# CloudEngineHub/PARC

Measured on AMD Instinct MI355X. Metric: env-steps/s, higher is better.
Workload: dtype f32; 1 GPU; full step (dynamics + obs/reward/done), 65536 envs total = 65536 per GPU, 5 bundled clips on a square blocky grid, reset of finished envs included; envs_per_gpu=65536, total_envs=65536, dynamics=True, parallelism=env-shard x1, launch=stream launches, library_abi=6

## Files before the change

parc_amd/csrc/parc_env.hip:

```cpp
#include <hip/hip_runtime.h>

#include <cmath>
#include <cstddef>
#include <cstdio>
#include <cstring>
#include <new>
#include <string>
#include <vector>

#include "../../include/parc_env.h"
#include "parc_common.hpp"
#include "parc_math.hpp"
#include "parc_dynamics.hpp"
#include "parc_dynamics_coop.hpp"
#include "parc_dynamics_wave.hpp"

using namespace parc;

#define REC_F4 32
#define REC_Q_POS 15
#define REC_Q_CONTACT 16
#define REC_Q_VEL 20

struct HierTables {
    float lt[16][3];
    float lr[16][4];
    int fk_paths[PARC_MAX_FK_PATHS][PARC_MAX_FK_DEPTH];
    int key_ids[8];
    int key_slot[16];
    int parent[16];
    int jtype[16];
    int dof_idx[16];
    float axis[16][4];
};
#define HIER_STAGED_WORDS ((int)(offsetof(HierTables, parent) / 4))

#define TILE_MAX_CELLS 320

struct DevTables {
    HierTables h;
    float tstep[8];
    float joint_err_w[16];
    float dof_err_w[PARC_MAX_DOFS];
    float contact_w[16];
    float pose_term_dist[16];
};

struct StepParams {
    int N, B, J, D, K, S, R, M, T;
    int lds_wave_floats;
    int global_obs, off_char;
    int lr_identity;
    int obs_tar, obs_contact;
    int obs_dim, off_dofvel, off_key, off_tar, tar_w, off_tarc, off_cc, off_hf;
    float dt_f, episode_length, min_obs_h, max_obs_h;
    float pose_w, vel_w, root_pos_w, root_vel_w, key_pos_w;
    float root_pos_term_sq, root_rot_term;
    int early_term, pose_term, track_root, track_root_h, tracking, body_pos_from_fk, never_done;
    unsigned fall_mask;
    float term_h;
    const float *hf; int X, Y; float min_x, min_y, dx, dy; int tile_r;
    float rdx, rdy;
    unsigned tile_mul;
    float tstep[8];
    const float4 *records; const MotionMeta *meta; const float *motion_offsets; const float *env_offsets;
    const float *ray_points; const DevTables *tables;
    unsigned char *ema_code;
    unsigned *stamp_out;
    float4 *prep;
    ParcEnvBuffers buf;
};

__device__ __forceinline__ Q4 joint_dof_to_rot(int type, const float *axis4, const float *dof) {
    if (type == PARC_JOINT_HINGE) return axis_angle_to_quat(mk3(axis4[0], axis4[1], axis4[2]), dof[0]);
    if (type == PARC_JOINT_SPHERICAL) return exp_map_to_quat(mk3(dof[0], dof[1], dof[2]));
    return mk4(0.f, 0.f, 0.f, 1.f);
}

__device__ __forceinline__ void joint_rot_to_dof(int type, const float *axis4, Q4 q, float *out) {
    if (type == PARC_JOINT_HINGE) {
        V3 axis; float angle;
        quat_to_axis_angle(q, axis, angle);
        float dot = axis4[0] * axis.x + axis4[1] * axis.y + axis4[2] * axis.z;
        if (dot < 0.f) angle = angle * -1.f;
        out[0] = angle;
    } else if (type == PARC_JOINT_SPHERICAL) {
        V3 e = quat_to_exp_map(q);
        out[0] = e.x; out[1] = e.y; out[2] = e.z;
    }
}

__device__ __forceinline__ float cell_float_rcp(float p, float mn, float d, float rd) {
    const float x = p - mn;
    const float q0 = x * rd;
    const float r = fmaf(-d, q0, x);
    return rintf(fmaf(r, rd, q0));
}
__device__ __forceinline__ int cell_index_rcp(float p, float mn, float d, float rd) {
    float f = cell_float_rcp(p, mn, d, rd);
    f = fminf(fmaxf(f, -1.0e9f), 1.0e9f);
    return (int)f;
}

__device__ __forceinline__ int cell_index(float p, float mn, float d) {
    float f = rintf((p - mn) / d);
    f = fminf(fmaxf(f, -1.0e9f), 1.0e9f);
    return (int)f;
}

__global__ __launch_bounds__(64) void k_dynamics(const parcdyn::DynModel *__restrict__ M, parcdyn::DynTerrain T, ParcEnvBuffers buf,
                                                 const float *__restrict__ action, const float *__restrict__ env_off, int N) {
    const int e = blockIdx.x * blockDim.x + threadIdx.x;
    if (e >= N) return;
    parcdyn::DynState S;
    S.root_pos = buf.char_root_pos + 3 * (size_t)e; S.root_rot = buf.char_root_rot + 4 * (size_t)e;
    S.root_vel = buf.char_root_vel + 3 * (size_t)e; S.root_ang_vel = buf.char_root_ang_vel + 3 * (size_t)e;
    S.dof_pos = buf.char_dof_pos + (size_t)M->D * e; S.dof_vel = buf.char_dof_vel + (size_t)M->D * e;
    S.contact_force = buf.contact_forces + (size_t)3 * M->B * e; S.body_pos = nullptr;
    parcdyn::dyn_control_step(*M, T, S, action + (size_t)M->D * e, env_off + 3 * (size_t)e);
}

__global__ __launch_bounds__(64) void k_env_prep(const StepParams P, const int64_t *__restrict__ env_ids,
                                                 const int *__restrict__ env_ids32, const int *__restrict__ count_dev, int count) {
    if (count_dev) count = *count_dev;
    const int it = blockIdx.x * 4 + (threadIdx.x >> 4), j = threadIdx.x & 15;
    if (it >= count || j >= P.B) return;
    const int e = env_ids ? (int)env_ids[it] : (env_ids32 ? env_ids32[it] : it);
    const DevTables *__restrict__ T = P.tables;
    float4 *out = P.prep + (size_t)e * 16;
    if (j == 0) {
        const float4 rr = *(const float4 *)(P.buf.char_root_rot + 4 * (size_t)e);
        const float heading = calc_heading(rr);
        const Q4 hinv = heading_quat_inv(heading);
        out[0] = make_float4(cosf(heading), sinf(heading), hinv.z, hinv.w);
    } else {
        const float *dof = P.buf.char_dof_pos + (size_t)e * P.D;
        const int ty = T->h.jtype[j], di = T->h.dof_idx[j];
        Q4 q = mk4(0.f, 0.f, 0.f, 1.f);
        if (ty == PARC_JOINT_HINGE) q = axis_angle_to_quat(mk3(T->h.axis[j][0], T->h.axis[j][1], T->h.axis[j][2]), dof[di]);
        else if (ty == PARC_JOINT_SPHERICAL) q = exp_map_to_quat(mk3(dof[di], dof[di + 1], dof[di + 2]));
        out[j] = q;
    }
}

#ifdef PARC_STAMPS
#define STAMP(i) do { if (lane == 0) s_stamp[i] = __builtin_readcyclecounter(); } while (0)
#else
#define STAMP(i) do { } while (0)
#endif
#define MODE_STEP 0
#define MODE_OBS 1
#define ENVS_PER_BLOCK 4
#define WAVE_SYNC() asm volatile("" ::: "memory")
#define RAY_UNROLL 8

__device__ __forceinline__ float wave_sum(float v) {
#pragma unroll
    for (int off = 32; off >= 1; off >>= 1) v = v + __shfl_xor(v, off, 64);
    return v;
}

template <int CTRL>
__device__ __forceinline__ float dpp_f32(float v) {
    return __int_as_float(__builtin_amdgcn_update_dpp(0, __float_as_int(v), CTRL, 0xf, 0xf, false));
}
__device__ __forceinline__ float row_sum16(float v) {
    v = v + dpp_f32<0x128>(v);
    v = v + dpp_f32<0x124>(v);
    v = v + dpp_f32<0x122>(v);
    v = v + dpp_f32<0x121>(v);
    return v;
}
__device__ __forceinline__ float lane_value(float v, int l) { return __int_as_float(__builtin_amdgcn_readlane(__float_as_int(v), l)); }

template <int MODE, bool MIRROR, bool LOCALROOT = false, bool OBSVAR = false>
__global__ __launch_bounds__(256, 5) void k_env_post(const StepParams P, const int64_t *__restrict__ env_ids,
                                                 const int *__restrict__ env_ids32, const int *__restrict__ count_dev, int count,
                                                 unsigned long long *bump_calls) {
    extern __shared__ __align__(16) float s_obs_all[];
    __shared__ int s_tab_raw[HIER_STAGED_WORDS];
    const HierTables &s_tab = *reinterpret_cast<const HierTables *>(s_tab_raw);
    __shared__ float4 s_q_all[ENVS_PER_BLOCK][8][16];
    __shared__ float4 s_lq_all[ENVS_PER_BLOCK][2][16];
    __shared__ float4 s_fk_all[ENVS_PER_BLOCK][80];
    __shared__ float s_cdofv_all[ENVS_PER_BLOCK][PARC_MAX_DOFS];
    __shared__ float4 s_refvel_all[ENVS_PER_BLOCK][12];
    __shared__ float s_refct_all[ENVS_PER_BLOCK][16];
    __shared__ float s_cfn_all[ENVS_PER_BLOCK][16];
    __shared__ float s_sc_all[ENVS_PER_BLOCK][16];
#ifdef PARC_STAMPS
    __shared__ unsigned long long s_stamp_all[ENVS_PER_BLOCK][16];
#endif
    const int wv = __builtin_amdgcn_readfirstlane((int)(threadIdx.x >> 6));
    const int lane = threadIdx.x & 63;
    const bool GLOBALOBS = OBSVAR && P.global_obs != 0;
    const int oc = OBSVAR ? P.off_char : 0;
    const bool TAROBS = !OBSVAR || P.obs_tar != 0;
    const bool CONTACTOBS = !OBSVAR || P.obs_contact != 0;
    float *s_obs = s_obs_all + (size_t)wv * P.lds_wave_floats;
    float4 (*s_q)[16] = s_q_all[wv];
    float4 (*s_lq)[16] = s_lq_all[wv];
    float4 *s_fk = s_fk_all[wv];
    float4 *s_cbp = s_lq[0];
    float *s_cdofv = s_cdofv_all[wv];
    float4 *s_refvel = s_refvel_all[wv];
    float *s_refct = s_refct_all[wv], *s_cfn = s_cfn_all[wv];
#ifdef PARC_STAMPS
    unsigned long long *s_stamp = s_stamp_all[wv];
#endif
    float *s_tile = (float *)s_fk;
    float4 (*s_br)[16] = reinterpret_cast<float4 (*)[16]>(s_obs + ((P.off_tarc + 3) & ~3));

    if (MODE == MODE_OBS && bump_calls && blockIdx.x == 0 && threadIdx.x == 0) *bump_calls += 1ull;
    if (count_dev) count = *count_dev;
    const int it = blockIdx.x * ENVS_PER_BLOCK + wv;
    if (it >= count) return;
    int e = env_ids ? (int)env_ids[it] : (env_ids32 ? env_ids32[it] : it);
    e = __builtin_amdgcn_readfirstlane(e);
    STAMP(0);

    const int B = P.B, D = P.D, S = P.S, K = P.K, J = P.J;
    const DevTables *__restrict__ T = P.tables;

    float *orow = P.buf.obs + (size_t)e * P.obs_dim;

    constexpr int HW = HIER_STAGED_WORDS;
    constexpr int HN = (HW + 63) / 64;
    int tabreg[HN];
#pragma unroll
    for (int i = 0; i < HN; ++i) { const int w = lane + 64 * i; tabreg[i] = w < HW ? ((const int *)&T->h)[w] : 0; }
    float dofv = 0.f;
    if (lane < D) dofv = P.buf.char_dof_vel[(size_t)e * D + lane];
    float aux0 = 0.f, aux1 = 0.f, aux2 = 0.f;
    {
        const float *src = nullptr;
        if (lane >= 32 && lane < 32 + B) src = P.buf.contact_forces + 3 * ((size_t)e * B + (lane - 32));
        else if (lane == 30) src = P.buf.char_root_vel + 3 * (size_t)e;
        else if (lane == 31) src = P.buf.char_root_ang_vel + 3 * (size_t)e;
        if (src) { aux0 = src[0]; aux1 = src[1]; aux2 = src[2]; }
    }
    const int qi = lane & 15;
    float4 prepq = make_float4(0.f, 0.f, 0.f, 1.f);
    if (lane < 16) prepq = P.prep[(size_t)e * 16 + lane];
    float2 rayp[RAY_UNROLL];
#pragma unroll
    for (int i = 0; i < RAY_UNROLL; ++i) {
        const int r = lane + 64 * i;
        rayp[i] = r < P.R ? ((const float2 *)P.ray_points)[r] : make_float2(0.f, 0.f);
    }

    const int mid = P.buf.motion_ids[e];
    const int tid = P.buf.terrain_ids[e];
    const float toff = P.buf.time_offsets[e];
    int ts = P.buf.timestep[e];
    if (MODE == MODE_STEP) ts += 1;
    const float time = P.dt_f * (float)ts;
    const float mt = time + toff;
    const MotionMeta meta = P.meta[mid];
    const float eox = P.env_offsets[3 * e + 0], eoy = P.env_offsets[3 * e + 1], eoz = P.env_offsets[3 * e + 2];
    const float *mo = P.motion_offsets + 2 * ((size_t)mid * P.T + tid);
    const float offx = mo[0] - eox, offy = mo[1] - eoy;
    const float *crp = P.buf.char_root_pos + 3 * (size_t)e;
    const float *crr = P.buf.char_root_rot + 4 * (size_t)e;
    const V3 root_pos = mk3(crp[0], crp[1], crp[2]);
    const Q4 root_rot = mk4(crr[0], crr[1], crr[2], crr[3]);
    const float gx = root_pos.x + eox, gy = root_pos.y + eoy, gz = root_pos.z + eoz;

    Blend myb;
    {
        const int sid = lane & 7;
        float t = mt;
#pragma unroll
        for (int q = 0; q < PARC_MAX_TAR_STEPS; ++q) t = (sid - 1 == q) ? mt + P.tstep[q] : t;
        myb = frame_blend(meta, t);
    }
    const int last_frame = meta.start + meta.nframes - 1;
    float4 fA[2], fB[2];
    Blend bl[2];
#pragma unroll
    for (int p = 0; p < 2; ++p) {
        const int r = p * 4 + (lane >> 4);
        const int src = max(r - 1, 0);
        bl[p].b = __shfl(myb.b, src, 64);
        bl[p].i0 = __shfl(myb.i0, src, 64);
        bl[p].i1 = min(bl[p].i0 + 1, last_frame);
        fA[p] = make_float4(0.f, 0.f, 0.f, 1.f); fB[p] = fA[p];
        if (r >= 1 && r < 2 + S) {
            fA[p] = P.records[(size_t)bl[p].i0 * REC_F4 + qi];
            fB[p] = P.records[(size_t)bl[p].i1 * REC_F4 + qi];
        }
    }
    float4 cA = make_float4(0.f, 0.f, 0.f, 0.f), cB = cA;
    float cblend = 0.f;
    const int nvel = 2 + (D + 3) / 4;
    {
        const int src = lane < 4 * (1 + S) ? lane >> 2 : 0;
        const float b2b = __shfl(myb.b, src, 64);
        const int b2i0 = __shfl(myb.i0, src, 64), b2i1 = min(b2i0 + 1, last_frame);
        if (lane < 4 * (1 + S)) {
            const int c = lane & 3;
            cblend = b2b;
            cA = P.records[(size_t)b2i0 * REC_F4 + REC_Q_CONTACT + c];
            cB = P.records[(size_t)b2i1 * REC_F4 + REC_Q_CONTACT + c];
        } else if (lane >= 32 && lane < 32 + nvel) {
            cA = P.records[(size_t)b2i0 * REC_F4 + REC_Q_VEL + (lane - 32)];
        }
    }
    const int tr = P.tile_r, TW = 2 * tr + 1, ncell = tr >= 0 ? TW * TW : 0;
    const int ox = min(max(cell_index(gx, P.min_x, P.dx) - tr, -(1 << 22)), 1 << 22), oy = min(max(cell_index(gy, P.min_y, P.dy) - tr, -(1 << 22)), 1 << 22);
    float tilev[5];
#pragma unroll
    for (int i = 0; i < 5; ++i) {
        const int idx = lane + 64 * i;
        tilev[i] = 0.f;
        if (idx < ncell) {
            const int a = (int)(((unsigned)idx * P.tile_mul) >> 16), bq = idx - a * TW;
            const int cx = min(max(ox + a, 0), P.X - 1), cy = min(max(oy + bq, 0), P.Y - 1);
            tilev[i] = P.hf[(size_t)cx * P.Y + cy];
        }
    }

    const float ch = __shfl(prepq.x, 0, 64), sh = __shfl(prepq.y, 0, 64);
    const Q4 hinv = mk4(0.f, 0.f, __shfl(prepq.z, 0, 64), __shfl(prepq.w, 0, 64));
#pragma unroll
    for (int i = 0; i < HN; ++i) { const int w = lane + 64 * i; if (w < HW) s_tab_raw[w] = tabreg[i]; }
    if (lane < D) {
        s_cdofv[lane] = dofv;
        s_obs[P.off_dofvel + lane] = dofv;
    }
    if (OBSVAR && oc && lane == 29) s_obs[0] = root_pos.z;
    if (lane == 30 || lane == 31) {
        const V3 r = GLOBALOBS ? mk3(aux0, aux1, aux2) : quat_rotate(hinv, mk3(aux0, aux1, aux2));
        const int o = oc + (lane == 30 ? 6 : 9);
        s_obs[o + 0] = r.x; s_obs[o + 1] = r.y; s_obs[o + 2] = r.z;
    }
    if (lane >= 32 && lane < 32 + B) {
        const float n = norm3(mk3(aux0, aux1, aux2));
        if (CONTACTOBS) orow[P.off_cc + (lane - 32)] = n > 1e-5f ? 1.f : 0.f;
        s_cfn[lane - 32] = fminf(n, 1.0f);
    }
#pragma unroll
    for (int i = 0; i < 5; ++i) { const int idx = lane + 64 * i; if (idx < ncell) s_tile[idx] = tilev[i]; }
    WAVE_SYNC();
    STAMP(1);

    {
        float *hrow = orow + P.off_hf;
        float *hmirror = MIRROR && P.buf.ray_hfs ? P.buf.ray_hfs + (size_t)e * P.R : nullptr;
        for (int base = 0; base < P.R; base += 64 * RAY_UNROLL) {
            if (base > 0) {
#pragma unroll
                for (int i = 0; i < RAY_UNROLL; ++i) { const int r = base + lane + 64 * i; rayp[i] = r < P.R ? ((const float2 *)P.ray_points)[r] : make_float2(0.f, 0.f); }
            }
            const float tlox = (float)ox, thix = (float)(ox + TW - 1), tloy = (float)oy, thiy = (float)(oy + TW - 1);
            if (tr >= 0) {
                int tix[RAY_UNROLL];
#pragma unroll
                for (int i = 0; i < RAY_UNROLL; ++i) {
                    tix[i] = 0;
                    if (base + 64 * i < P.R) {
                        const float px = (rayp[i].x * ch - rayp[i].y * sh) + gx;
                        const float py = (rayp[i].x * sh + rayp[i].y * ch) + gy;
                        const int a = (int)fminf(fmaxf(cell_float_rcp(px, P.min_x, P.dx, P.rdx), tlox), thix) - ox;
                        const int bq = (int)fminf(fmaxf(cell_float_rcp(py, P.min_y, P.dy, P.rdy), tloy), thiy) - oy;
                        tix[i] = a * TW + bq;
                    }
                    asm volatile("" : "+v"(tix[i]));
                }
                float hv[RAY_UNROLL];
#pragma unroll
                for (int i = 0; i < RAY_UNROLL; ++i) hv[i] = s_tile[tix[i]];
#pragma unroll
                for (int i = 0; i < RAY_UNROLL; ++i) {
                    const int r = base + lane + 64 * i;
                    if (r < P.R) {
                        float h = hv[i] - gz;
                        h = fminf(fmaxf(h, P.min_obs_h), P.max_obs_h);
                        hrow[r] = h;
                        if (hmirror) hmirror[r] = h;
                    }
                }
            } else {
#pragma unroll
                for (int i = 0; i < RAY_UNROLL; ++i) {
                    const int r = base + lane + 64 * i;
                    if (r < P.R) {
                        const float px = (rayp[i].x * ch - rayp[i].y * sh) + gx;
                        const float py = (rayp[i].x * sh + rayp[i].y * ch) + gy;
                        const int ix = cell_index_rcp(px, P.min_x, P.dx, P.rdx), iy = cell_index_rcp(py, P.min_y, P.dy, P.rdy);
                        const int cx = min(max(ix, 0), P.X - 1), cy = min(max(iy, 0), P.Y - 1);
                        float h = P.hf[(size_t)cx * P.Y + cy] - gz;
                        h = fminf(fmaxf(h, P.min_obs_h), P.max_obs_h);
                        hrow[r] = h;
                        if (hmirror) hmirror[r] = h;
                    }
                }
            }
        }
    }
    STAMP(2);

#pragma unroll
    for (int p = 0; p < 2; ++p) {
        const int r = p * 4 + (lane >> 4);
        const int i = qi;
        if (r < 2 + S) {
            float4 res = make_float4(0.f, 0.f, 0.f, 1.f);
            if (r == 0) {
                if (i == 0) res = root_rot;
                else if (i == 15) res = make_float4(root_pos.x, root_pos.y, root_pos.z, 0.f);
                else if (i < B) res = prepq;
            } else {
                const float4 A = fA[p], Bv = fB[p];
                const float bb = bl[p].b;
                if (i == 15) {
                    const float a = 1.0f - bb;
                    res.x = a * A.x + bb * Bv.x;
                    res.y = a * A.y + bb * Bv.y;
                    res.z = a * A.z + bb * Bv.z;
                    res.w = 0.f;
                    if (meta.loop == PARC_LOOP_WRAP) {
                        float t = mt;
#pragma unroll
                        for (int q = 0; q < PARC_MAX_TAR_STEPS; ++q) t = (r - 2 == q) ? mt + P.tstep[q] : t;
                        const float ph = floorf(t / meta.length);
                        res.x = res.x + ph * meta.dx; res.y = res.y + ph * meta.dy; res.z = res.z + ph * meta.dz;
                    }
                    res.x = res.x + offx;
                    res.y = res.y + offy;
                } else if (i < B) {
                    res = slerp_rr(A, Bv, bb);
                }
            }
            if (i >= 1 && i < B) {
                const Q4 lq = P.lr_identity ? res : quat_mul(mk4(s_tab.lr[i][0], s_tab.lr[i][1], s_tab.lr[i][2], s_tab.lr[i][3]), res);
                if (r < 2) { s_lq[r][i] = lq; s_q[r][i] = res; } else s_q[r][i] = lq;
            } else {
                s_q[r][i] = res;
            }
            if (r == 1) {
                if (MIRROR && i == 0 && P.buf.ref_root_rot) *(float4 *)(P.buf.ref_root_rot + 4 * (size_t)e) = res;
                if (MIRROR && i >= 1 && i < B && P.buf.ref_joint_rot) *(float4 *)(P.buf.ref_joint_rot + 4 * ((size_t)e * J + i - 1)) = res;
                if (MIRROR && i == 15 && P.buf.ref_root_pos) {
                    float *o = P.buf.ref_root_pos + 3 * (size_t)e;
                    o[0] = res.x; o[1] = res.y; o[2] = res.z;
                }
            } else if (r == 0 || TAROBS) {
                const int base = r == 0 ? 0 : P.off_tar + (r - 2) * P.tar_w;
                if (i < B) {
                    const Q4 qq = (i == 0 && !GLOBALOBS) ? quat_mul(hinv, res) : res;
                    float tn[6];
                    quat_to_tan_norm(qq, tn);
                    const int o = r == 0 ? oc + (i == 0 ? 0 : 12 + 6 * (i - 1)) : base + 3 + 6 * i;
#pragma unroll
                    for (int c = 0; c < 6; ++c) s_obs[o + c] = tn[c];
                } else if (i == 15 && r >= 2) {
                    const V3 rpd = mk3(res.x - root_pos.x, res.y - root_pos.y, res.z - root_pos.z);
                    const V3 rpo = GLOBALOBS ? rpd : quat_rotate(hinv, rpd);
                    s_obs[base + 0] = rpo.x; s_obs[base + 1] = rpo.y; s_obs[base + 2] = rpo.z;
                }
            }
        }
    }
    if (lane < 4 * (1 + S)) {
        const int s = lane >> 2, c = lane & 3;
        const float b = cblend, a = 1.0f - b;
        const float v[4] = {a * cA.x + b * cB.x, a * cA.y + b * cB.y, a * cA.z + b * cB.z, a * cA.w + b * cB.w};
#pragma unroll
        for (int k = 0; k < 4; ++k) {
            const int bd = 4 * c + k;
            if (bd < B) {
                if (s == 0) {
                    s_refct[bd] = v[k];
                    if (MIRROR && P.buf.ref_contacts) P.buf.ref_contacts[(size_t)e * B + bd] = v[k];
                } else if (TAROBS && CONTACTOBS) {
                    orow[P.off_tarc + (s - 1) * B + bd] = v[k];
                }
            }
        }
    } else if (lane >= 32 && lane < 32 + nvel) {
        const int c = lane - 32;
        s_refvel[c] = cA;
        if (MIRROR && c == 0 && P.buf.ref_root_vel) { float *o = P.buf.ref_root_vel + 3 * (size_t)e; o[0] = cA.x; o[1] = cA.y; o[2] = cA.z; }
        if (MIRROR && c == 1 && P.buf.ref_root_ang_vel) { float *o = P.buf.ref_root_ang_vel + 3 * (size_t)e; o[0] = cA.x; o[1] = cA.y; o[2] = cA.z; }
        if (MIRROR && c >= 2 && P.buf.ref_dof_vel) {
            const float vv[4] = {cA.x, cA.y, cA.z, cA.w};
            for (int k = 0; k < 4; ++k) { const int d = 4 * (c - 2) + k; if (d < D) P.buf.ref_dof_vel[(size_t)e * D + d] = vv[k]; }
        }
    }
    float bpx = 0.f, bpy = 0.f, bpz = 0.f;
    if (!P.body_pos_from_fk && lane < B) {
        const float *src = P.buf.char_body_pos + 3 * ((size_t)e * B + lane);
        bpx = src[0]; bpy = src[1]; bpz = src[2];
    }
    WAVE_SYNC();
    STAMP(3);

    {
        const int k = lane >> 3, c = lane & 7;
        if (k < 2 + S) {
            Q4 prot = s_q[k][0];
            const float4 *jq = k < 2 ? s_lq[k] : s_q[k];
            const float4 pp = s_q[k][15];
            V3 ppos = mk3(pp.x, pp.y, pp.z);
            if (c == 0 && k < 2) {
                s_fk[k * 16] = make_float4(ppos.x, ppos.y, ppos.z, 0.f);
                if (MIRROR && P.tracking) s_br[k][0] = prot;
            }
#pragma unroll 1
            for (int d = 0; d < PARC_MAX_FK_DEPTH; ++d) {
                const int b = s_tab.fk_paths[c][d];
                if (b < 0) break;
                const V3 wt = quat_rotate(prot, mk3(s_tab.lt[b][0], s_tab.lt[b][1], s_tab.lt[b][2]));
                ppos = mk3(ppos.x + wt.x, ppos.y + wt.y, ppos.z + wt.z);
                prot = quat_mul(prot, jq[b]);
                if (k < 2) {
                    s_fk[k * 16 + b] = make_float4(ppos.x, ppos.y, ppos.z, 0.f);
                    if (MIRROR && P.tracking) s_br[k][b] = prot;
                } else {
                    const int slot = s_tab.key_slot[b];
                    if (slot >= 0) s_fk[32 + (k - 2) * 8 + slot] = make_float4(ppos.x, ppos.y, ppos.z, 0.f);
                }
            }
        }
    }
    WAVE_SYNC();
    if (lane < B) s_cbp[lane] = P.body_pos_from_fk ? s_fk[lane] : make_float4(bpx, bpy, bpz, 0.f);
    STAMP(4);

    if (lane < 8 * (1 + S)) {
        const int row = lane >> 3, kk = lane & 7;
        if (kk < K) {
            if (row == 0) {
                const float4 kp = s_fk[s_tab.key_ids[kk]];
                const V3 rd = mk3(kp.x - root_pos.x, kp.y - root_pos.y, kp.z - root_pos.z);
                const V3 rl = GLOBALOBS ? rd : quat_rotate(hinv, rd);
                const int o = P.off_key + 3 * kk;
                s_obs[o] = rl.x; s_obs[o + 1] = rl.y; s_obs[o + 2] = rl.z;
            } else if (TAROBS) {
                const int r = row + 1;
                const float4 kp = s_fk[32 + (r - 2) * 8 + s_tab.key_slot[s_tab.key_ids[kk]]], trp = s_q[r][15];
                const V3 rd = mk3(kp.x - trp.x, kp.y - trp.y, kp.z - trp.z);
                const int tb = P.off_tar + (r - 2) * P.tar_w, o = tb + 3 + 6 * B + 3 * kk;
                if (GLOBALOBS) {
                    s_obs[o] = rd.x; s_obs[o + 1] = rd.y; s_obs[o + 2] = rd.z;
                } else {
                    const V3 rl = quat_rotate(hinv, rd);
                    s_obs[o] = rl.x + s_obs[tb]; s_obs[o + 1] = rl.y + s_obs[tb + 1]; s_obs[o + 2] = rl.z + s_obs[tb + 2];
                }
            }
        }
    }
    STAMP(5);

    if (MODE == MODE_STEP) {
        {
            float *sc = s_sc_all[wv];
            bool fc = false;
            if (P.fall_mask != 0u && lane >= 32 && lane < 32 + B && !((P.fall_mask >> (lane - 32)) & 1u))
                fc = fabsf(aux0) > 0.1f || fabsf(aux1) > 0.1f || fabsf(aux2) > 0.1f;
            const bool fcany = __ballot(fc) != 0ull;
            if (lane == 30) { sc[5] = aux0; sc[6] = aux1; sc[7] = aux2; }
            if (lane == 31) { sc[8] = aux0; sc[9] = aux1; sc[10] = aux2; }
            if (lane == 0) {
                sc[0] = time; sc[1] = mt; sc[2] = __int_as_float(ts); sc[3] = meta.length; sc[4] = __int_as_float(meta.loop);
                sc[11] = fcany ? 1.f : 0.f; sc[12] = eox; sc[13] = eoy; sc[14] = __int_as_float(e);
            }
        }
        asm volatile("s_waitcnt lgkmcnt(0)\n\ts_barrier" ::: "memory");
        const int nact = min(ENVS_PER_BLOCK, count - (int)blockIdx.x * ENVS_PER_BLOCK);
        int owner = blockIdx.x & (ENVS_PER_BLOCK - 1);
        if (owner >= nact) owner = 0;
        if (wv == owner) {
            const int j = lane >> 4, i = lane & 15, rowbase = lane & 48;
            const bool valid = j < nact;
            const int jj = valid ? j : 0;
            const float4 (*q)[16] = s_q_all[jj];
            const float4 *fk = s_fk_all[jj];
            const float4 *cbp = s_lq_all[jj][0];
            const float *scj = s_sc_all[jj];
            const float4 rp4 = q[0][15], trp = q[1][15];
            float dang = 0.f, vpose = 0.f;
            Q4 hinv_c = mk4(0.f, 0.f, 0.f, 1.f), hinv_r = hinv_c;
            if (LOCALROOT) {
                hinv_c = heading_quat_inv(calc_heading(q[0][0]));
                hinv_r = heading_quat_inv(calc_heading(q[1][0]));
            }
            if (i <= J) {
                const int slot = i < J ? 1 + i : 0;
                if (LOCALROOT) {
                    Q4 qa = q[0][slot], qb = q[1][slot];
                    if (i == J) { qa = quat_mul(hinv_c, qa); qb = quat_mul(hinv_r, qb); }
                    dang = quat_diff_angle(qa, qb);
                } else {
                    dang = quat_diff_angle(q[0][slot], q[1][slot]);
                }
                if (i < J) vpose = T->joint_err_w[i] * dang * dang;
            }
            float vs[4] = {0.f, 0.f, 0.f, 0.f};
#pragma unroll
            for (int pss = 0; pss < (PARC_MAX_DOFS + 15) / 16; ++pss) {
                if (16 * pss < D) {
                    const int d = 16 * pss + i;
                    float v = 0.f;
                    if (d < D) {
                        const float dv = ((const float *)s_refvel_all[jj])[8 + d] - s_cdofv_all[jj][d];
                        v = T->dof_err_w[d] * dv * dv;
                    }
                    vs[pss] = row_sum16(v);
                }
            }
            float vkey = 0.f;
            if (i < K) {
                const int b = s_tab.key_ids[i];
                const float4 kp = cbp[b], tk = fk[16 + b];
                if (LOCALROOT) {
                    const V3 kt = quat_rotate(hinv_r, mk3(tk.x - trp.x, tk.y - trp.y, tk.z - trp.z));
                    const V3 kc = quat_rotate(hinv_c, mk3(kp.x - rp4.x, kp.y - rp4.y, kp.z - rp4.z));
                    const float dx = kt.x - kc.x, dy = kt.y - kc.y, dz = kt.z - kc.z;
                    vkey = dx * dx + dy * dy + dz * dz;
                } else {
                    const float dx = (tk.x - trp.x) - (kp.x - rp4.x);
                    const float dy = (tk.y - trp.y) - (kp.y - rp4.y);
                    const float dz = (tk.z - trp.z) - (kp.z - rp4.z);
                    vkey = dx * dx + dy * dy + dz * dz;
                }
            }
            float vct = 0.f;
            if (i < B) {
                const float tar = s_refct_all[jj][i], f = s_cfn_all[jj][i];
                float cr = -(1.0f - tar) * f;
                cr = cr + tar * f;
                vct = T->contact_w[i] * cr;
            }
            bool bad = false;
            if (i >= 1 && i < B) {
                const float4 bp = cbp[i], b0 = cbp[0], tp = fk[16 + i], t0 = fk[16];
                const float dx = (tp.x - t0.x) - (bp.x - b0.x);
                const float dy = (tp.y - t0.y) - (bp.y - b0.y);
                const float dz = (tp.z - t0.z) - (bp.z - b0.z);
                const float lim = T->pose_term_dist[i - 1];
                bad = (dx * dx + dy * dy + dz * dz) > lim * lim;
            }
            const bool pose_fail_any = ((unsigned)(__ballot(bad) >> rowbase) & 0xffffu) != 0u;
            bool fallen = false;
            if (P.fall_mask != 0u) {
                bool fh = false;
                if (i < B && !((P.fall_mask >> i) & 1u)) {
                    const float4 bp = cbp[i];
                    const int ix = min(max(cell_index(bp.x + scj[12], P.min_x, P.dx), 0), P.X - 1), iy = min(max(cell_index(bp.y + scj[13], P.min_y, P.dy), 0), P.Y - 1);
                    fh = bp.z < P.hf[(size_t)ix * P.Y + iy] + P.term_h;
                }
                fallen = scj[11] != 0.f && ((unsigned)(__ballot(fh) >> rowbase) & 0xffffu) != 0u;
            }
            const float root_rot_angle = __shfl(dang, rowbase + J, 64);
            const float pose_err = __shfl(row_sum16(vpose), rowbase, 64), csum = __shfl(row_sum16(vct), rowbase, 64), key_err = __shfl(row_sum16(vkey), rowbase, 64);
            const float vel_err = __shfl((vs[0] + vs[1]) + (vs[2] + vs[3]), rowbase, 64);

            const float time_j = scj[0], mt_j = scj[1], mlen_j = scj[3];
            const int ts_j = __float_as_int(scj[2]), mloop_j = __float_as_int(scj[4]), e_j = __float_as_int(scj[14]);
            float rdx = trp.x - rp4.x, rdy = trp.y - rp4.y, rdz = trp.z - rp4.z;
            if (!P.track_root) { rdx = 0.f; rdy = 0.f; }
            if (!P.track_root_h) rdz = 0.f;
            const float root_pos_err = rdx * rdx + rdy * rdy + rdz * rdz;
            const float4 tv = s_refvel_all[jj][0], tav = s_refvel_all[jj][1];
            const float rre = root_rot_angle * root_rot_angle;
            float rve, rave;
            if (LOCALROOT) {
                const V3 tv3 = quat_rotate(hinv_r, mk3(tv.x, tv.y, tv.z)), tav3 = quat_rotate(hinv_r, mk3(tav.x, tav.y, tav.z));
                const V3 rv3 = quat_rotate(hinv_c, mk3(scj[5], scj[6], scj[7])), rav3 = quat_rotate(hinv_c, mk3(scj[8], scj[9], scj[10]));
                float d0 = tv3.x - rv3.x, d1 = tv3.y - rv3.y, d2 = tv3.z - rv3.z;
                rve = d0 * d0 + d1 * d1 + d2 * d2;
                d0 = tav3.x - rav3.x; d1 = tav3.y - rav3.y; d2 = tav3.z - rav3.z;
                rave = d0 * d0 + d1 * d1 + d2 * d2;
            } else {
// ... 709 lines not shown
        size_t end = all.find(';', at);
        if (end == std::string::npos) end = all.size();
        if (all.compare(at, k.size(), k) == 0) return all.substr(at + k.size(), end - at - k.size());
        at = end + 1;
    }
    return "";
}

static int wave_envs_per_block(int N, int num_cus) { return (N + 63) / 64 <= num_cus / 2 ? 32 : 64; }

struct ParcEnv {
    ParcEnvConfig cfg;
    int B, J, D, K, S, R, N, M = 0, T = 1;
    int obs_dim;
    int64_t F = 0;
    bool bound = false, have_motions = false, have_terrain = false;
    bool done_list_fresh = false;
    StepParams sp;
    float4 *d_prep = nullptr;
    std::string dev_options_s, describe_s;
    unsigned int *h_health = nullptr, *d_health = nullptr;
    float *d_man_ovf = nullptr;
    float *d_root_shadow = nullptr;
    parcdyn::DynModel h_dyn;
    parcdyn::DynModel *d_dyn = nullptr;
    parcdyn::CoopTables h_coop;
    parcdyn::CoopTables *d_coop = nullptr;
    bool use_coop = false;
    parcdyn::WaveTables h_wave;
    parcdyn::WaveTables *d_wave = nullptr;
    bool use_wave = false, wave_rejected = false;
    DevTables h_tab;
    DevTables *d_tab = nullptr;
    float *d_ray = nullptr, *d_env_off = nullptr, *d_hf = nullptr, *d_motion_off = nullptr;
    float4 *d_records = nullptr;
    MotionMeta *d_meta = nullptr;
    std::vector<MotionMeta> h_meta;
    std::vector<float> h_weights;
    float *d_weights = nullptr, *d_fail = nullptr, *d_cdf = nullptr;
    unsigned char *d_ema = nullptr;
    int *d_done_list = nullptr, *d_done_key = nullptr, *d_chunk_count = nullptr, *d_motion_done = nullptr, *d_reset_count = nullptr;
    int nchunks = 0;
    float *d_scratch_jr = nullptr, *d_start_frac = nullptr;
    RenderGeoms *d_rgeom = nullptr;
    float hf_max = 0.f;
    float hf_min = 0.f;
    char *d_scene = nullptr;
    int scene_cap = 0;
    unsigned long long *d_reset_calls = nullptr;
    const float *action_bound = nullptr;
    hipGraphExec_t graph_exec = nullptr;
    bool graph_dirty = true;
    bool force_ema_leader = false;
    bool force_two_launch_curriculum = false;
    int grid_waves = 0;
    int num_cus = 256;
    size_t lds_bytes = 0;
    float last_dyn_ms = 0.f;
    hipEvent_t ev[4] = {nullptr, nullptr, nullptr, nullptr};
    float *rec_frames = nullptr, *rec_obs = nullptr;
    int rec_cap = 0, rec_ref = 0;
    int *rec_count = nullptr, *rec_nwriting = nullptr;
    unsigned char *rec_writing = nullptr;
    bool timing = false;
    std::vector<hipEvent_t> tev;
    size_t tev_used = 0;
};

extern "C" const char *parc_last_error(void) { return g_err.c_str(); }
extern "C" int parc_abi_version(void) { return PARC_ABI_VERSION; }

static void free_dev(ParcEnv *e) {
    void *ptrs[] = {e->d_man_ovf, e->d_root_shadow, e->d_prep, e->d_dyn, e->d_coop, e->d_wave, e->d_tab, e->d_ray, e->d_env_off, e->d_hf, e->d_motion_off, e->d_records, e->d_meta, e->d_weights, e->d_fail,
                    e->d_cdf, e->d_ema, e->d_done_list, e->d_done_key, e->d_chunk_count, e->d_motion_done, e->d_reset_count, e->d_reset_calls,
                    e->d_scratch_jr, e->d_rgeom, e->d_scene};
    for (void *p : ptrs) if (p) (void)hipFree(p);
    if (e->h_health) (void)hipHostFree(e->h_health);
    for (auto &ev : e->ev) if (ev) (void)hipEventDestroy(ev);
    for (auto &ev : e->tev) if (ev) (void)hipEventDestroy(ev);
    if (e->graph_exec) (void)hipGraphExecDestroy(e->graph_exec);
}

static int sync_params(ParcEnv *e) {
    e->graph_dirty = true;
    return PARC_OK;
}

extern "C" int parc_env_create(const ParcEnvConfig *cfg, ParcEnv **out) {
    if (!cfg || !out) return fail(PARC_ERR_INVALID, "null argument");
    if (cfg->abi_version != PARC_ABI_VERSION || cfg->struct_size != sizeof(ParcEnvConfig))
        return fail(PARC_ERR_INVALID, "ParcEnvConfig ABI mismatch (abi_version / struct_size)");
    const ParcCharModel &m = cfg->model;
    if (m.num_bodies < 2 || m.num_bodies > 15) return fail(PARC_ERR_INVALID, "num_bodies must be in [2,15]");
    if (m.dof_size < 1 || m.dof_size > PARC_MAX_DOFS) return fail(PARC_ERR_INVALID, "dof_size must be in [1,40]");
    if (cfg->num_tar_obs_steps < 1 || cfg->num_tar_obs_steps > PARC_MAX_TAR_STEPS) return fail(PARC_ERR_INVALID, "tar_obs_steps: 1..6 entries");
    if (cfg->num_key_bodies < 0 || cfg->num_key_bodies > PARC_MAX_KEY_BODIES) return fail(PARC_ERR_INVALID, "key_bodies: at most 8");
    if (cfg->num_envs < 1) return fail(PARC_ERR_INVALID, "num_envs must be >= 1");
    if (cfg->num_rays < 1 || cfg->num_rays > 4096 || !cfg->ray_points_host) return fail(PARC_ERR_INVALID, "ray fan: 1..4096 points");
    if (!cfg->env_offsets_host) return fail(PARC_ERR_INVALID, "env_offsets_host is required");
    for (int b = 1; b < m.num_bodies; ++b)
        if (m.parent[b] < 0 || m.parent[b] >= b) return fail(PARC_ERR_INVALID, "bodies must be in DFS order (parent < child)");
    if (cfg->enable_dynamics && !cfg->body_pos_from_fk)
        return fail(PARC_ERR_INVALID, "enable_dynamics needs body_pos_from_fk = 1 (the simulator is reduced-coordinate)");
    if (cfg->enable_dynamics && (cfg->dynamics.num_geoms < 1 || cfg->dynamics.num_geoms > PARC_MAX_GEOMS || !(cfg->dynamics.sim_dt > 0.f)))
        return fail(PARC_ERR_INVALID, "enable_dynamics: bad ParcDynamicsParams");

    int ndev = 0;
    if (hipGetDeviceCount(&ndev) != hipSuccess || ndev <= 0) return fail(PARC_ERR_NO_DEVICE, "no HIP device visible");
    if (cfg->device < 0 || cfg->device >= ndev) return fail(PARC_ERR_INVALID, "device ordinal out of range");
    HIPCHK(hipSetDevice(cfg->device));

    ParcEnv *e = new (std::nothrow) ParcEnv();
    if (!e) return fail(PARC_ERR_INVALID, "out of host memory");
    e->cfg = *cfg;
    e->dev_options_s = cfg->dev_options ? cfg->dev_options : "";
    e->cfg.dev_options = e->dev_options_s.c_str();
    e->cfg.ray_points_host = nullptr; e->cfg.env_offsets_host = nullptr;
    e->B = m.num_bodies; e->J = e->B - 1; e->D = m.dof_size; e->K = cfg->num_key_bodies; e->S = cfg->num_tar_obs_steps;
    e->R = cfg->num_rays; e->N = cfg->num_envs;
    const int B = e->B, J = e->J, D = e->D, K = e->K, S = e->S, R = e->R;

    DevTables &t = e->h_tab;
    memset(&t, 0, sizeof(t));
    for (int b = 0; b < 16; ++b) { t.h.parent[b] = -1; t.h.jtype[b] = PARC_JOINT_FIXED; t.h.key_slot[b] = -1; }
    for (int b = 0; b < B; ++b) {
        t.h.parent[b] = m.parent[b]; t.h.jtype[b] = m.joint_type[b]; t.h.dof_idx[b] = m.dof_idx[b];
        for (int c = 0; c < 3; ++c) { t.h.axis[b][c] = m.joint_axis[b][c]; t.h.lt[b][c] = m.local_translation[b][c]; }
        for (int c = 0; c < 4; ++c) t.h.lr[b][c] = m.local_rotation[b][c];
    }
    for (int p = 0; p < PARC_MAX_FK_PATHS; ++p)
        for (int d = 0; d < PARC_MAX_FK_DEPTH; ++d) {
            t.h.fk_paths[p][d] = m.fk_paths[p][d];
            if (m.fk_paths[p][d] >= B) { delete e; return fail(PARC_ERR_INVALID, "fk_paths entry out of range"); }
        }
    const float dt_f = (float)cfg->control_dt;
    for (int s = 0; s < S; ++s) t.tstep[s] = dt_f * (float)cfg->tar_obs_steps[s];
    for (int k = 0; k < K; ++k) {
        if (cfg->key_body_ids[k] < 0 || cfg->key_body_ids[k] >= B) { delete e; return fail(PARC_ERR_INVALID, "key body id out of range"); }
        t.h.key_ids[k] = cfg->key_body_ids[k];
        if (t.h.key_slot[cfg->key_body_ids[k]] < 0) t.h.key_slot[cfg->key_body_ids[k]] = k;
    }
    for (int j = 0; j < J; ++j) { t.joint_err_w[j] = cfg->joint_err_w[j]; t.pose_term_dist[j] = cfg->pose_termination_dist[j]; }
    for (int d = 0; d < D; ++d) t.dof_err_w[d] = cfg->dof_err_w[d];
    for (int b = 0; b < B; ++b) t.contact_w[b] = cfg->contact_weights[b];

    StepParams &sp = e->sp;
    memset(&sp, 0, sizeof(sp));
    sp.N = e->N; sp.B = B; sp.J = J; sp.D = D; sp.K = K; sp.S = S; sp.R = R;
    sp.global_obs = cfg->global_obs; sp.off_char = cfg->global_root_height_obs ? 1 : 0;
    sp.off_dofvel = sp.off_char + 12 + 6 * J;
    sp.off_key = sp.off_dofvel + D;
    sp.off_tar = sp.off_key + 3 * K;
    sp.tar_w = 3 + 6 + 6 * J + 3 * K;
    sp.lr_identity = 1;
    for (int b = 0; b < B; ++b)
        if (!(cfg->model.local_rotation[b][0] == 0.f && cfg->model.local_rotation[b][1] == 0.f && cfg->model.local_rotation[b][2] == 0.f && cfg->model.local_rotation[b][3] == 1.f)) sp.lr_identity = 0;
    sp.obs_tar = cfg->enable_tar_obs != 0; sp.obs_contact = cfg->use_contact_info != 0;
    sp.off_tarc = sp.off_tar + (sp.obs_tar ? S * sp.tar_w : 0);
    sp.off_cc = sp.off_tarc + (sp.obs_tar && sp.obs_contact ? S * B : 0);
    sp.off_hf = sp.off_cc + (sp.obs_contact ? B : 0);
    sp.obs_dim = sp.off_hf + R;
    e->obs_dim = sp.obs_dim;
    for (int q = 0; q < S; ++q) sp.tstep[q] = dt_f * (float)cfg->tar_obs_steps[q];
    sp.dt_f = dt_f; sp.episode_length = cfg->episode_length; sp.min_obs_h = cfg->min_obs_h; sp.max_obs_h = cfg->max_obs_h;
    sp.pose_w = cfg->pose_w; sp.vel_w = cfg->vel_w; sp.root_pos_w = cfg->root_pos_w; sp.root_vel_w = cfg->root_vel_w; sp.key_pos_w = cfg->key_pos_w;
    sp.root_pos_term_sq = (float)((double)cfg->root_pos_termination_dist * (double)cfg->root_pos_termination_dist);
    sp.root_rot_term = cfg->root_rot_termination_angle;
    sp.early_term = cfg->enable_early_termination; sp.pose_term = cfg->pose_termination; sp.track_root = cfg->track_root;
    sp.track_root_h = cfg->track_root_h; sp.tracking = cfg->report_tracking_error; sp.body_pos_from_fk = cfg->body_pos_from_fk;
    sp.fall_mask = cfg->contact_body_mask & ((1u << B) - 1u); sp.term_h = cfg->termination_height;

    auto up = [&](void **dst, const void *src, size_t bytes) -> hipError_t {
        hipError_t r = hipMalloc(dst, bytes);
        if (r != hipSuccess) return r;
        return src ? hipMemcpy(*dst, src, bytes, hipMemcpyHostToDevice) : hipMemset(*dst, 0, bytes);
    };
    hipError_t r = hipSuccess;
    const size_t N = (size_t)e->N;
    if ((r = up((void **)&e->d_tab, &t, sizeof(t))) != hipSuccess ||
        (r = up((void **)&e->d_prep, nullptr, sizeof(float4) * 16 * N)) != hipSuccess ||
        (r = up((void **)&e->d_ray, cfg->ray_points_host, sizeof(float) * 2 * R)) != hipSuccess ||
        (r = up((void **)&e->d_env_off, cfg->env_offsets_host, sizeof(float) * 3 * N)) != hipSuccess ||
        (r = up((void **)&e->d_ema, nullptr, ((N + 1023) / 1024) * 1024)) != hipSuccess ||
        (r = up((void **)&e->d_done_list, nullptr, sizeof(int) * N)) != hipSuccess ||
        (r = up((void **)&e->d_done_key, nullptr, sizeof(int) * N)) != hipSuccess ||
        (r = up((void **)&e->d_chunk_count, nullptr, sizeof(int) * 1024)) != hipSuccess ||
        (r = up((void **)&e->d_reset_count, nullptr, 2 * sizeof(int))) != hipSuccess ||
        (r = up((void **)&e->d_reset_calls, nullptr, sizeof(unsigned long long))) != hipSuccess ||
        (r = up((void **)&e->d_scratch_jr, nullptr, sizeof(float) * 4 * J * N)) != hipSuccess) {
        free_dev(e); delete e;
        return fail(PARC_ERR_HIP, std::string("device allocation failed: ") + hipGetErrorString(r));
    }
    {
        RenderGeoms rg;
        memset(&rg, 0, sizeof(rg));
        const ParcDynamicsParams &dp = cfg->dynamics;
        for (int g = 0; g < dp.num_geoms && g < PARC_MAX_GEOMS; ++g) {
            if (dp.geom_body[g] < 0 || dp.geom_body[g] >= B || dp.geom_type[g] < PARC_GEOM_BOX || dp.geom_type[g] > PARC_GEOM_CAPSULE) continue;
            const int n = rg.n++;
            rg.body[n] = dp.geom_body[g]; rg.type[n] = dp.geom_type[g];
            for (int c = 0; c < 3; ++c) { rg.p0[n][c] = dp.geom_pos[g][c]; rg.p1[n][c] = dp.geom_pos2[g][c]; rg.size[n][c] = dp.geom_size[g][c]; }
        }
        r = up((void **)&e->d_rgeom, &rg, sizeof(rg));
    }
    if (r != hipSuccess) {
        free_dev(e); delete e;
        return fail(PARC_ERR_HIP, std::string("device allocation failed: ") + hipGetErrorString(r));
    }
    {
        hipDeviceProp_t prop;
        (void)hipGetDeviceProperties(&prop, cfg->device);
        e->grid_waves = prop.multiProcessorCount * 16;
        e->num_cus = prop.multiProcessorCount;
    }
    if (cfg->enable_dynamics) {
        memset(&e->h_dyn, 0, sizeof(e->h_dyn));
        parcdyn::fill_dyn_model(e->h_dyn, cfg->model, cfg->dynamics, cfg->action_low, cfg->action_high);
        if (e->h_dyn.truncated > 0 || cfg->dynamics.num_geoms > PARC_MAX_GEOMS) {
            const int t = e->h_dyn.truncated;
            free_dev(e); delete e;
            return fail(PARC_ERR_INVALID, "dynamics: " + std::to_string(t) + " collision point(s) / segment(s) / geom(s) do not fit the model tables (DYN_MAXC " +
                        std::to_string(DYN_MAXC) + ", DYN_MAXS " + std::to_string(DYN_MAXS) + ", " + std::to_string(PARC_MAX_GEOMS) + " geoms)");
        }
        {
            const int cm = cfg->dynamics.control_mode;
            bool all_1d = true;
            for (int b = 1; b < cfg->model.num_bodies; ++b) all_1d = all_1d && cfg->model.joint_type[b] != parcdyn::DJ_SPHERICAL;
            if (cm < PARC_CTRL_PD || cm > PARC_CTRL_PD_1D || (cm == PARC_CTRL_PD_1D && !all_1d)) {
                free_dev(e); delete e;
                return fail(PARC_ERR_INVALID, cm == PARC_CTRL_PD_1D ? "control_mode pd_1d only supports characters whose joints all have one dof (the reference asserts it, ig_char_env.py:246-250)"
                                                                     : "unknown control_mode " + std::to_string(cm));
            }
        }
        {
            const std::string mode = dev_opt(cfg, "segments");
            if (!mode.empty()) {
                parcdyn::DynModel &dm = e->h_dyn;
                int keep = 0;
                for (int k = 0; k < dm.nseg; ++k) {
                    const bool drop = mode == "none" || (mode == "capsules" && dm.seg_r[k] <= 0.011f);
                    if (drop) continue;
                    dm.seg_body[keep] = dm.seg_body[k]; dm.seg_r[keep] = dm.seg_r[k];
                    for (int a = 0; a < 3; ++a) { dm.seg_a[keep][a] = dm.seg_a[k][a]; dm.seg_b[keep][a] = dm.seg_b[k][a]; }
                    ++keep;
                }
                dm.nseg = keep;
            }
            const std::string dt_ = dev_opt(cfg, "dtang");
            if (!dt_.empty()) e->h_dyn.dtang = (float)atof(dt_.c_str());
            const std::string mp_ = dev_opt(cfg, "man_period");
            if (!mp_.empty() && atoi(mp_.c_str()) >= 1) {
                e->h_dyn.man_period = atoi(mp_.c_str());
                e->h_dyn.spec_tv = 1.5f * (float)(e->h_dyn.man_period - 1) * e->h_dyn.dt;
            }
        }
        if ((r = up((void **)&e->d_dyn, &e->h_dyn, sizeof(e->h_dyn))) != hipSuccess) {
            free_dev(e); delete e;
            return fail(PARC_ERR_HIP, std::string("device allocation failed: ") + hipGetErrorString(r));
        }
        const std::string want = dev_opt(cfg, "kernel");
        const bool coop_ok = parcdyn::build_coop_tables(e->h_dyn, e->h_coop);
        const bool wave_ok = coop_ok && parcdyn::build_wave_tables(e->h_dyn, e->h_coop, e->h_wave);
        e->wave_rejected = !wave_ok;
        e->use_wave = wave_ok && want != "coop" && want != "thread";
        e->use_coop = coop_ok && !e->use_wave && want != "thread";
        if (e->use_wave) {
            r = up((void **)&e->d_wave, &e->h_wave, sizeof(e->h_wave));
            if (r == hipSuccess && dev_opt(cfg, "no_residual").empty()) {
                r = hipMalloc((void **)&e->d_root_shadow, sizeof(float) * 6 * N);
                if (r == hipSuccess) r = hipMemset(e->d_root_shadow, 0xff, sizeof(float) * 6 * N);
            }
            if (r == hipSuccess) {
                const int epb = wave_envs_per_block(N, e->num_cus);
                r = hipMalloc((void **)&e->d_man_ovf, sizeof(float) * (size_t)((N + epb - 1) / epb) * WV_MAXLIMB * WV_MAN_OVF * 8 * 64);
            }
            if (r == hipSuccess)
                r = hipFuncSetAttribute(cfg->dynamics.control_mode == PARC_CTRL_PD ? (const void *)parcdyn::k_dynamics_wave : (const void *)parcdyn::k_dynamics_wave_ff,
                                        hipFuncAttributeMaxDynamicSharedMemorySize, parcdyn::wv_lds_floats() * (int)sizeof(float));
        } else if (e->use_coop) {
            r = up((void **)&e->d_coop, &e->h_coop, sizeof(e->h_coop));
        }
        if (r != hipSuccess) {
            free_dev(e); delete e;
            return fail(PARC_ERR_HIP, std::string("dynamics kernel setup failed: ") + hipGetErrorString(r));
        }
    }
    e->force_ema_leader = !dev_opt(cfg, "ema_leader").empty();
    e->force_two_launch_curriculum = !dev_opt(cfg, "curriculum_two_launches").empty();
    if (hipHostMalloc((void **)&e->h_health, 2 * sizeof(unsigned int), hipHostMallocMapped) == hipSuccess) {
        e->h_health[0] = 0u; e->h_health[1] = 0u;
        if (hipHostGetDevicePointer((void **)&e->d_health, e->h_health, 0) != hipSuccess) e->d_health = nullptr;
    }
    for (auto &ev : e->ev) (void)hipEventCreate(&ev);
    sp.tables = e->d_tab; sp.ray_points = e->d_ray; sp.env_offsets = e->d_env_off;
    sp.ema_code = e->d_ema; sp.prep = e->d_prep;
#ifdef PARC_STAMPS
    if (hipMalloc((void **)&sp.stamp_out, sizeof(unsigned) * 8 * N) != hipSuccess) sp.stamp_out = nullptr;
#endif
    e->nchunks = (e->N + 1023) / 1024;
    if (e->nchunks > 1024) { free_dev(e); delete e; return fail(PARC_ERR_INVALID, "num_envs must be <= 1048576 per handle"); }

    *out = e;
    return PARC_OK;
}

extern "C" void parc_env_destroy(ParcEnv *e) {
// ... 1016 lines not shown
```

Before: 99.08 million env-steps/s.

## Pack reference row items densely across lanes and trim redundant FK quaternion multiplies

Replaces the fixed lane-to-(row, body) mapping, in which each of up to eight rows took 16 lanes, with a dense item map. The first 16 lanes handle root rotation and position for each row, and the remaining lanes enumerate joint items row by row using a multiply-shift division. This cuts the idle lanes in the two blend and observation passes and lets pass B specialise to joint-only work. The FK loop also prefetches the next path entry and skips the final quaternion multiply when it is not needed. In exchange it adds index arithmetic, a host-side multiplier check, and more complex branching.

```diff
diff --git a/parc_amd/csrc/parc_env.hip b/parc_amd/csrc/parc_env.hip
--- a/parc_amd/csrc/parc_env.hip
+++ b/parc_amd/csrc/parc_env.hip
@@ -6,11 +6,13 @@
 #include <cstring>
 #include <new>
 #include <string>
+#include <type_traits>
 #include <vector>
 
 #include "../../include/parc_env.h"
 #include "parc_common.hpp"
 #include "parc_math.hpp"
+#include "parc_rowmap.hpp"
 #include "parc_dynamics.hpp"
 #include "parc_dynamics_coop.hpp"
 #include "parc_dynamics_wave.hpp"
@@ -62,6 +64,7 @@
     const float *hf; int X, Y; float min_x, min_y, dx, dy; int tile_r;
     float rdx, rdy;
     unsigned tile_mul;
+    unsigned row_mul;
     float tstep[8];
     const float4 *records; const MotionMeta *meta; const float *motion_offsets; const float *env_offsets;
     const float *ray_points; const DevTables *tables;
@@ -239,9 +242,9 @@
         else if (lane == 31) src = P.buf.char_root_ang_vel + 3 * (size_t)e;
         if (src) { aux0 = src[0]; aux1 = src[1]; aux2 = src[2]; }
     }
-    const int qi = lane & 15;
+    const int item[2] = {parc_rowmap_item<true>(lane, B, 2 + S, P.row_mul), parc_rowmap_item<false>(lane, B, 2 + S, P.row_mul)};
     float4 prepq = make_float4(0.f, 0.f, 0.f, 1.f);
-    if (lane < 16) prepq = P.prep[(size_t)e * 16 + lane];
+    if ((unsigned)item[0] < 15u) prepq = P.prep[(size_t)e * 16 + item[0]];
     float2 rayp[RAY_UNROLL];
 #pragma unroll
     for (int i = 0; i < RAY_UNROLL; ++i) {
@@ -279,15 +282,15 @@
     Blend bl[2];
 #pragma unroll
     for (int p = 0; p < 2; ++p) {
-        const int r = p * 4 + (lane >> 4);
+        const int r = max(item[p], 0) >> 4;
         const int src = max(r - 1, 0);
         bl[p].b = __shfl(myb.b, src, 64);
         bl[p].i0 = __shfl(myb.i0, src, 64);
         bl[p].i1 = min(bl[p].i0 + 1, last_frame);
         fA[p] = make_float4(0.f, 0.f, 0.f, 1.f); fB[p] = fA[p];
-        if (r >= 1 && r < 2 + S) {
-            fA[p] = P.records[(size_t)bl[p].i0 * REC_F4 + qi];
-            fB[p] = P.records[(size_t)bl[p].i1 * REC_F4 + qi];
+        if (r >= 1) {
+            fA[p] = P.records[(size_t)bl[p].i0 * REC_F4 + (item[p] & 15)];
+            fB[p] = P.records[(size_t)bl[p].i1 * REC_F4 + (item[p] & 15)];
         }
     }
     float4 cA = make_float4(0.f, 0.f, 0.f, 0.f), cB = cA;
@@ -400,68 +403,69 @@
     }
     STAMP(2);
 
-#pragma unroll
-    for (int p = 0; p < 2; ++p) {
-        const int r = p * 4 + (lane >> 4);
-        const int i = qi;
-        if (r < 2 + S) {
-            float4 res = make_float4(0.f, 0.f, 0.f, 1.f);
-            if (r == 0) {
-                if (i == 0) res = root_rot;
-                else if (i == 15) res = make_float4(root_pos.x, root_pos.y, root_pos.z, 0.f);
-                else if (i < B) res = prepq;
+    static_assert(2 * (PARC_MAX_BODIES - 2) <= PARC_ROWMAP_JOINTS_A, "the joints of rows 0 and 1 must fit into pass A");
+    auto row_pass = [&](auto root_tag, const int itm, const float4 A, const float4 Bv, const float bb) {
+        constexpr bool ROOT = decltype(root_tag)::value;
+        if (itm < 0) return;
+        const int r = itm >> 4, i = itm & 15;
+        const bool is_rot = ROOT && i == 0, is_pos = ROOT && i == 15;
+        const bool row0 = ROOT && r == 0, row1 = ROOT && r == 1;
+        float4 res = make_float4(0.f, 0.f, 0.f, 1.f);
+        if (row0) {
+            if (is_rot) res = root_rot;
+            else if (is_pos) res = make_float4(root_pos.x, root_pos.y, root_pos.z, 0.f);
+            else res = prepq;
+        } else {
+            if (is_pos) {
+                const float a = 1.0f - bb;
+                res.x = a * A.x + bb * Bv.x;
+                res.y = a * A.y + bb * Bv.y;
+                res.z = a * A.z + bb * Bv.z;
+                res.w = 0.f;
+                if (meta.loop == PARC_LOOP_WRAP) {
+                    float t = mt;
+#pragma unroll
+                    for (int q = 0; q < PARC_MAX_TAR_STEPS; ++q) t = (r - 2 == q) ? mt + P.tstep[q] : t;
+                    const float ph = floorf(t / meta.length);
+                    res.x = res.x + ph * meta.dx; res.y = res.y + ph * meta.dy; res.z = res.z + ph * meta.dz;
+                }
+                res.x = res.x + offx;
+                res.y = res.y + offy;
             } else {
-                const float4 A = fA[p], Bv = fB[p];
-                const float bb = bl[p].b;
-                if (i == 15) {
-                    const float a = 1.0f - bb;
-                    res.x = a * A.x + bb * Bv.x;
-                    res.y = a * A.y + bb * Bv.y;
-                    res.z = a * A.z + bb * Bv.z;
-                    res.w = 0.f;
-                    if (meta.loop == PARC_LOOP_WRAP) {
-                        float t = mt;
-#pragma unroll
-                        for (int q = 0; q < PARC_MAX_TAR_STEPS; ++q) t = (r - 2 == q) ? mt + P.tstep[q] : t;
-                        const float ph = floorf(t / meta.length);
-                        res.x = res.x + ph * meta.dx; res.y = res.y + ph * meta.dy; res.z = res.z + ph * meta.dz;
-                    }
-                    res.x = res.x + offx;
-                    res.y = res.y + offy;
-                } else if (i < B) {
-                    res = slerp_rr(A, Bv, bb);
-                }
-            }
-            if (i >= 1 && i < B) {
-                const Q4 lq = P.lr_identity ? res : quat_mul(mk4(s_tab.lr[i][0], s_tab.lr[i][1], s_tab.lr[i][2], s_tab.lr[i][3]), res);
-                if (r < 2) { s_lq[r][i] = lq; s_q[r][i] = res; } else s_q[r][i] = lq;
-            } else {
-                s_q[r][i] = res;
-            }
-            if (r == 1) {
-                if (MIRROR && i == 0 && P.buf.ref_root_rot) *(float4 *)(P.buf.ref_root_rot + 4 * (size_t)e) = res;
-                if (MIRROR && i >= 1 && i < B && P.buf.ref_joint_rot) *(float4 *)(P.buf.ref_joint_rot + 4 * ((size_t)e * J + i - 1)) = res;
-                if (MIRROR && i == 15 && P.buf.ref_root_pos) {
-                    float *o = P.buf.ref_root_pos + 3 * (size_t)e;
-                    o[0] = res.x; o[1] = res.y; o[2] = res.z;
-                }
-            } else if (r == 0 || TAROBS) {
-                const int base = r == 0 ? 0 : P.off_tar + (r - 2) * P.tar_w;
-                if (i < B) {
-                    const Q4 qq = (i == 0 && !GLOBALOBS) ? quat_mul(hinv, res) : res;
-                    float tn[6];
-                    quat_to_tan_norm(qq, tn);
-                    const int o = r == 0 ? oc + (i == 0 ? 0 : 12 + 6 * (i - 1)) : base + 3 + 6 * i;
-#pragma unroll
-                    for (int c = 0; c < 6; ++c) s_obs[o + c] = tn[c];
-                } else if (i == 15 && r >= 2) {
-                    const V3 rpd = mk3(res.x - root_pos.x, res.y - root_pos.y, res.z - root_pos.z);
-                    const V3 rpo = GLOBALOBS ? rpd : quat_rotate(hinv, rpd);
-                    s_obs[base + 0] = rpo.x; s_obs[base + 1] = rpo.y; s_obs[base + 2] = rpo.z;
-                }
-            }
-        }
-    }
+                res = slerp_rr(A, Bv, bb);
+            }
+        }
+        if (!is_rot && !is_pos) {
+            const Q4 lq = P.lr_identity ? res : quat_mul(mk4(s_tab.lr[i][0], s_tab.lr[i][1], s_tab.lr[i][2], s_tab.lr[i][3]), res);
+            if (row0 || row1) { s_lq[r][i] = lq; s_q[r][i] = res; } else s_q[r][i] = lq;
+        } else {
+            s_q[r][i] = res;
+        }
+        if (row1) {
+            if (MIRROR && is_rot && P.buf.ref_root_rot) *(float4 *)(P.buf.ref_root_rot + 4 * (size_t)e) = res;
+            if (MIRROR && !is_rot && !is_pos && P.buf.ref_joint_rot) *(float4 *)(P.buf.ref_joint_rot + 4 * ((size_t)e * J + i - 1)) = res;
+            if (MIRROR && is_pos && P.buf.ref_root_pos) {
+                float *o = P.buf.ref_root_pos + 3 * (size_t)e;
+                o[0] = res.x; o[1] = res.y; o[2] = res.z;
+            }
+        } else if (row0 || TAROBS) {
+            const int base = row0 ? 0 : P.off_tar + (r - 2) * P.tar_w;
+            if (!is_pos) {
+                const Q4 qq = (is_rot && !GLOBALOBS) ? quat_mul(hinv, res) : res;
+                float tn[6];
+                quat_to_tan_norm(qq, tn);
+                const int o = row0 ? oc + (is_rot ? 0 : 12 + 6 * (i - 1)) : base + 3 + 6 * i;
+#pragma unroll
+                for (int c = 0; c < 6; ++c) s_obs[o + c] = tn[c];
+            } else if (!row0) {
+                const V3 rpd = mk3(res.x - root_pos.x, res.y - root_pos.y, res.z - root_pos.z);
+                const V3 rpo = GLOBALOBS ? rpd : quat_rotate(hinv, rpd);
+                s_obs[base + 0] = rpo.x; s_obs[base + 1] = rpo.y; s_obs[base + 2] = rpo.z;
+            }
+        }
+    };
+    row_pass(std::true_type(), item[0], fA[0], fB[0], bl[0].b);
+    row_pass(std::false_type(), item[1], fA[1], fB[1], bl[1].b);
     if (lane < 4 * (1 + S)) {
         const int s = lane >> 2, c = lane & 3;
         const float b = cblend, a = 1.0f - b;
@@ -507,13 +511,13 @@
                 s_fk[k * 16] = make_float4(ppos.x, ppos.y, ppos.z, 0.f);
                 if (MIRROR && P.tracking) s_br[k][0] = prot;
             }
+            int b = s_tab.fk_paths[c][0];
 #pragma unroll 1
-            for (int d = 0; d < PARC_MAX_FK_DEPTH; ++d) {
-                const int b = s_tab.fk_paths[c][d];
-                if (b < 0) break;
+            for (int d = 0; d < PARC_MAX_FK_DEPTH && b >= 0; ++d) {
+                const int nb = d + 1 < PARC_MAX_FK_DEPTH ? s_tab.fk_paths[c][d + 1] : -1;
                 const V3 wt = quat_rotate(prot, mk3(s_tab.lt[b][0], s_tab.lt[b][1], s_tab.lt[b][2]));
                 ppos = mk3(ppos.x + wt.x, ppos.y + wt.y, ppos.z + wt.z);
-                prot = quat_mul(prot, jq[b]);
+                if (nb >= 0 || (MIRROR && P.tracking)) prot = quat_mul(prot, jq[b]);
                 if (k < 2) {
                     s_fk[k * 16 + b] = make_float4(ppos.x, ppos.y, ppos.z, 0.f);
                     if (MIRROR && P.tracking) s_br[k][b] = prot;
@@ -521,6 +525,7 @@
                     const int slot = s_tab.key_slot[b];
                     if (slot >= 0) s_fk[32 + (k - 2) * 8 + slot] = make_float4(ppos.x, ppos.y, ppos.z, 0.f);
                 }
+                b = nb;
             }
         }
     }
@@ -1536,6 +1541,8 @@
     sp.off_key = sp.off_dofvel + D;
     sp.off_tar = sp.off_key + 3 * K;
     sp.tar_w = 3 + 6 + 6 * J + 3 * K;
+    sp.row_mul = parc_rowmap_mul(B);
+    if (!parc_rowmap_mul_ok(B, sp.row_mul)) { delete e; return fail(PARC_ERR_INVALID, "internal: row item multiplier"); }
     sp.lr_identity = 1;
     for (int b = 0; b < B; ++b)
         if (!(cfg->model.local_rotation[b][0] == 0.f && cfg->model.local_rotation[b][1] == 0.f && cfg->model.local_rotation[b][2] == 0.f && cfg->model.local_rotation[b][3] == 1.f)) sp.lr_identity = 0;
diff --git a/parc_amd/csrc/parc_rowmap.hpp b/parc_amd/csrc/parc_rowmap.hpp
--- /dev/null
+++ b/parc_amd/csrc/parc_rowmap.hpp
@@ -0,0 +1,28 @@
+#pragma once
+
+#if defined(__HIPCC__)
+#define PARC_ROWMAP_HD __host__ __device__ __forceinline__
+#else
+#define PARC_ROWMAP_HD inline
+#endif
+
+#define PARC_ROWMAP_ROOT_LANES 16
+#define PARC_ROWMAP_JOINTS_A (64 - PARC_ROWMAP_ROOT_LANES)
+#define PARC_ROWMAP_MAX_JOINT_ITEMS (PARC_ROWMAP_JOINTS_A + 64)
+
+PARC_ROWMAP_HD unsigned parc_rowmap_mul(int B) { return B > 1 ? (65536u + (unsigned)(B - 1) - 1u) / (unsigned)(B - 1) : 0u; }
+
+PARC_ROWMAP_HD bool parc_rowmap_mul_ok(int B, unsigned mul) {
+    if (B <= 1) return true;
+    for (unsigned j = 0; j < PARC_ROWMAP_MAX_JOINT_ITEMS; ++j)
+        if (((j * mul) >> 16) != j / (unsigned)(B - 1)) return false;
+    return true;
+}
+
+template <bool ROOT_ITEMS>
+PARC_ROWMAP_HD int parc_rowmap_item(int lane, int B, int rows, unsigned mul) {
+    if (ROOT_ITEMS && lane < PARC_ROWMAP_ROOT_LANES) return (lane & 7) < rows ? 16 * (lane & 7) + (lane < 8 ? 0 : 15) : -1;
+    const int j = ROOT_ITEMS ? lane - PARC_ROWMAP_ROOT_LANES : lane + PARC_ROWMAP_JOINTS_A;
+    const int row = (int)(((unsigned)j * mul) >> 16);
+    return j < rows * (B - 1) ? 16 * row + 1 + (j - row * (B - 1)) : -1;
+}
```

Measured after the change: 100.8 million env-steps/s (median of 6 runs). 1.7% higher.
